# KolinGuo/MPlib

Measured on AMD Instinct MI355X. Metric: configs/sec full collide() Panda-7DoF+10 boxes, higher is better.
Workload: dtype f64; 1 GPU; cfg3 panda_10boxes: 1048576 configs/GPU/step, 129 pairs, full self+world collide() with ACM filter; configs_per_gpu=1048576, pairs=129, mask_words=5, parallelism=dp1 (config shards, no data-path collective)

## Files before the change

### mplib_amd/csrc/mpg_abi_world.h

```cpp
#pragma once

const char* mpg_last_error(void) { return g_last_error.c_str(); }

int mpg_fcl_bvh_build(const double* vertices, int32_t n_vertices, const int32_t* triangles, int32_t n_triangles,
                      double* boxes, int32_t* links, int32_t* leaf_order) {
  if (n_triangles <= 0 || !vertices || !triangles || !boxes || !links || !leaf_order)
    return set_error(MPG_E_INVALID, "mpg_fcl_bvh_build: empty mesh or NULL buffer");
  for (int64_t i = 0; i < 3 * (int64_t)n_triangles; ++i)
    if (triangles[i] < 0 || triangles[i] >= n_vertices) return set_error(MPG_E_INVALID, "triangle vertex out of range");
  FclBvh B;
  B.box.resize(FB_STRIDE);
  B.link.resize(3);
  std::vector<int> prim((size_t)n_triangles);
  for (int t = 0; t < n_triangles; ++t) prim[t] = t;
  fcl_bvh_node(B, vertices, triangles, prim, 0, 0, n_triangles, 0);
  std::copy(B.box.begin(), B.box.end(), boxes);
  std::copy(B.link.begin(), B.link.end(), links);
  std::copy(prim.begin(), prim.end(), leaf_order);
  return (int)(B.link.size() / 3);
}

int mpg_last_error_copy(char* buf, size_t size) {
  const size_t len = g_last_error.size();
  if (buf && size > 0) {
// ... 71 lines not shown

int mpg_synchronize(int device) {
  HIP_TRY(hipSetDevice(device));
  HIP_TRY(hipDeviceSynchronize());
  return MPG_OK;
}

int mpg_world_create(const mpg_world_desc* d_in, int device, mpg_world** out) {
  if (!out) return set_error(MPG_E_INVALID, "out is NULL");
  *out = nullptr;
  int rc = validate(d_in);
  if (rc) return rc;
  mpg_world_desc dd = *d_in;
  std::vector<int32_t> lp_kin(dd.link_parent, dd.link_parent + dd.n_links);
  int n_free = 0;
  for (int32_t& p : lp_kin)
    if (p == MPG_LINK_FREE) {
      p = 0;
      ++n_free;
    }
  if (n_free) dd.link_parent = lp_kin.data();
  const mpg_world_desc* d = &dd;
  std::vector<double> geom_rec((size_t)G_STRIDE * std::max(d->n_geoms, 1), 0.0);
  for (int g = 0; g < d->n_geoms; ++g) geom_record(d, g, geom_rec.data() + (size_t)G_STRIDE * g);
  std::vector<double> obb((size_t)7 * std::max(d->n_geoms, 1), 0.0);
  for (int g = 0; g < d->n_geoms; ++g) {
    const double* r = geom_rec.data() + (size_t)G_STRIDE * g;
    for (int k = 0; k < 3; ++k) obb[7 * g + k] = r[G_OBB_C + k];
    for (int k = 0; k < 3; ++k) obb[7 * g + 3 + k] = r[G_OBB_E + k];
    obb[7 * g + 6] = r[G_RADIUS];
  }
  BpProgram bpp;
  bp_build(d, obb, bpp);
  size_t lds = 0;
  const int W = std::max(1, (d->n_pairs + 31) / 32);
  const int block = choose_block(cull_lds_per_thread(d->n_moving, bpp.n_saves, W), &lds);
  if (block < 0) return set_error(MPG_E_UNSUPPORTED, "world too large for the phase-A LDS budget");
  HIP_TRY(hipSetDevice(device));

  std::vector<double> static_rec((size_t)S_STRIDE * std::max(d->n_static, 1), 0.0);
  for (int s = 0; s < d->n_static; ++s) static_record(d, s, geom_rec.data(), static_rec.data() + (size_t)S_STRIDE * s);
  std::vector<int> gstart(std::max(d->n_geoms, 1), 0), ngroups(std::max(d->n_geoms, 1), 0);
  std::vector<double> hull;
  std::vector<int> cbase(std::max(d->n_geoms, 1), -1), geom_nbr(std::max(d->n_geoms, 1), -1), hull_nbr, wcell_end, wcell_end2, wcell_pre;
  std::vector<double> cell_rec, cell_ovf, wcell_rec, wcell_ovf, wcell_aux, nbr_ent;
  const int walk_subk =
      std::getenv("MPG_WALK_SUBK") ? std::max(1, std::min(8, std::atoi(std::getenv("MPG_WALK_SUBK")))) : kSubK;
  int big_words = 0;
  for (int g = 0; g < d->n_geoms; ++g) {
    if (d->geom_type[g] != MPG_GEOM_CONVEX) continue;
    const double* Vg = d->vertices + 3 * (size_t)d->geom_vertex_start[g];
    const int nvg = d->geom_vertex_count[g];
    std::vector<int> enc;
    const int nf = (int)d->geom_param[4 * g + 1];
    bool walk = nf > 0 && fcl_convex_neighbors(nvg, d->convex_face + (int64_t)d->geom_param[4 * g], nf, enc);
#ifdef MPG_DIAG
    if (std::getenv("MPG_DEBUG_NO_WALK")) walk = false;
#endif
    if (walk) {
      geom_nbr[g] = (int)(hull_nbr.size() / 2);
      if (nvg > kMaxWalkVerts) big_words = std::max(big_words, (nvg + 63) / 64);
      for (int i = 0; i < nvg; ++i) {
        const int st = enc[i], cnt = enc[st];
        hull_nbr.push_back((int)(nbr_ent.size() / 4));
        hull_nbr.push_back(cnt);
        for (int k = 1; k <= cnt; ++k) {
// ... 406 lines not shown
  const size_t o_al = bb.add(allowed.data(), allowed.size());
  const size_t o_cf = bb.add(pair_cf.data(), pair_cf.size());
  const size_t o_sT = bb.add(d->static_transform, 12 * (size_t)d->n_static);
  const size_t o_cs = bb.add(chain_start.data(), chain_start.size());
  const size_t o_cl = bb.add(chain_len.data(), chain_len.size());
  const size_t o_cj = bb.add(chain_joints.data(), chain_joints.size());
  const size_t o_ss = bb.add(sched_start.data(), sched_start.size());
  const size_t o_sp = bb.add(sched_pair.data(), sched_pair.size());
  const size_t o_so = bb.add(sched_other.data(), sched_other.size());
  const size_t o_sts = bb.add(st_start.data(), st_start.size());
  const size_t o_stm = bb.add(st_m.data(), st_m.size());
  const size_t o_str = bb.add(st_r.data(), st_r.size());
  const size_t o_pbd = bb.add(prism_bound.data(), prism_bound.size());
  const size_t o_amk = bb.add(all_mask.data(), all_mask.size());
  const size_t o_bjs = bb.add(bpp.jsrc.data(), bpp.jsrc.size());
  const size_t o_bjv = bb.add(bpp.jsave.data(), bpp.jsave.size());
  const size_t o_bja = bb.add(bpp.jaxis.data(), bpp.jaxis.size());
  const size_t o_bjp = bb.add(bpp.jplace.data(), bpp.jplace.size());
  const size_t o_bls = bb.add(bpp.link_start.data(), bpp.link_start.size());
  const size_t o_blo = bb.add(bpp.link_order.data(), bpp.link_order.size());
  const size_t o_blp = bb.add(bpp.lplace.data(), bpp.lplace.size());
  const size_t o_bos = bb.add(bpp.obj_start.data(), bpp.obj_start.size());
  const size_t o_boo = bb.add(bpp.obj_order.data(), bpp.obj_order.size());
  const size_t o_bmo = bb.add(bpp.moff.data(), bpp.moff.size());
  const size_t o_bmb = bb.add(bpp.mobj.data(), bpp.mobj.size());
  const size_t o_bsb = bb.add(bpp.sobj.data(), bpp.sobj.size());
  if (bpp.jobj_order.empty()) bpp.jobj_order.push_back(0);
  const size_t o_bjk = bb.add(bpp.jkind.data(), bpp.jkind.size());
  const size_t o_bjo = bb.add(bpp.jobj_start.data(), bpp.jobj_start.size());
  const size_t o_bjr = bb.add(bpp.jobj_order.data(), bpp.jobj_order.size());
  const size_t o_bop = bb.add(bpp.oplace.data(), bpp.oplace.size());
  const size_t o_boq = bb.add(bpp.oquat.data(), bpp.oquat.size());
  const size_t o_boc = bb.add(bpp.ocen.data(), bpp.ocen.size());
  const size_t o_olf = bb.add(oct_leaf.data(), oct_leaf.size());
  const size_t o_mtr = bb.add(mesh_tri.data(), mesh_tri.size());
  const size_t o_mnd = bb.add(mesh_node.data(), mesh_node.size());
  const size_t o_mln = bb.add(mesh_link.data(), mesh_link.size());
  const size_t o_mtt = bb.add(mesh_tree.data(), mesh_tree.size());
  const size_t o_lrec = bb.add(lat_rec.data(), lat_rec.size());
  const size_t o_fbb = bb.add(fbvh.box.data(), fbvh.box.size());
  const size_t o_fbl = bb.add(fbvh.link.data(), fbvh.link.size());
  const size_t o_fbr = bb.add(fb_root.data(), fb_root.size());
  const size_t o_tps = bb.add(tri_pos.data(), tri_pos.size());
  const size_t o_sob = bb.add(sobb.data(), sobb.size());
  const size_t o_ogr = bb.add(oct_grid.data(), oct_grid.size());
  const size_t o_oce = bb.add(oct_cells.data(), oct_cells.size());
  const size_t o_oli = bb.add(oct_list.data(), oct_list.size());
  const size_t o_opa = bb.add(oct_path.data(), oct_path.size());
  const size_t o_ode = bb.add(oct_depth.data(), oct_depth.size());
  std::vector<int> free_obj(n_free, 0);
  for (int m = 0; m < d->n_moving; ++m)
    if (d->moving_link[m] >= d->n_links - n_free) free_obj[d->moving_link[m] - (d->n_links - n_free)] = m;
  const size_t o_fob = n_free ? bb.add(free_obj.data(), free_obj.size()) : 0;

  std::unique_ptr<mpg_world> w(new mpg_world());
  w->device = device;
  w->n_geoms = d->n_geoms;
  w->geom_type_h.assign(d->geom_type, d->geom_type + d->n_geoms);
  w->block = block;
  w->lds_bytes = lds;
  w->blob_bytes = bb.bytes.size();
  {
    uint64_t h = 1469598103934665603ull;
    for (const char c : bb.bytes) h = (h ^ (uint8_t)c) * 1099511628211ull;
    w->snapshot_hash = h;
  }
  HIP_TRY(w->blob.reserve(w->blob_bytes));
  HIP_TRY(hipMemcpy(w->blob.get(), bb.bytes.data(), w->blob_bytes, hipMemcpyHostToDevice));
  char* base = w->blob.get();
  DevWorld& dw = w->dw;
  dw.nj = d->n_joints;
  dw.dof = d->dof;
  dw.n_links = d->n_links;
  dw.n_geoms = d->n_geoms;
  dw.n_moving = d->n_moving;
  dw.n_static = d->n_static;
  dw.n_pairs = d->n_pairs;
  dw.W = W;
  dw.mpr_tol = d->gjk_tolerance;
  dw.bp_margin = bp_margin;
  dw.small_margin = small_margin;
  dw.n_prism = n_prism;
  dw.prism_bound = to_cptr<double>(base + o_pbd);
  dw.pose_bound = pose_bound;
  dw.all_mask = to_cptr<int>(base + o_amk);
  dw.n_free = n_free;
  dw.far_r = far_r;
  dw.free_obj = to_cptr<int>(base + o_fob);
  dw.free_cur = nullptr;
  if (n_free) {
    w->free_host.resize((size_t)n_free * 7);
    for (int k = 0; k < n_free; ++k) {
      const double* lp = d->link_placement + 12 * (size_t)(d->n_links - n_free + k);
      double* p7 = w->free_host.data() + 7 * (size_t)k;
      for (int i = 0; i < 3; ++i) p7[i] = lp[9 + i];
      mat_to_quat(lp, &p7[3], &p7[4]);
    }
    HIP_TRY(w->free_dev.reserve(w->free_host.size()));
    HIP_TRY(hipMemcpy(w->free_dev.get(), w->free_host.data(), sizeof(double) * w->free_host.size(),
                      hipMemcpyHostToDevice));
    dw.free_cur = w->free_dev.get();
  }
#ifdef MPG_DIAG
  if (const char* m = std::getenv("MPG_DEBUG_MARGIN")) {
    dw.bp_margin = (float)std::atof(m);
    dw.small_margin = std::atof(m);
  }
#endif
  dw.debug_mode = 0;
#ifdef MPG_DIAG
  if (const char* e = std::getenv("MPG_DEBUG_CULL")) dw.debug_mode = std::atoi(e);
#endif
  dw.big_vis = nullptr;
  dw.big_busy = nullptr;
  dw.big_slots = 0;
  dw.big_words = big_words;
  if (big_words > 0) {
    dw.big_slots = 8192;
    HIP_TRY(w->big_vis.reserve((size_t)dw.big_slots * big_words));
    dw.big_vis = w->big_vis.get();
    HIP_TRY(hipMemset(dw.big_vis, 0, sizeof(unsigned long long) * (size_t)dw.big_slots * big_words));
    HIP_TRY(w->big_busy.reserve((size_t)dw.big_slots));
    dw.big_busy = w->big_busy.get();
    HIP_TRY(hipMemset(dw.big_busy, 0, sizeof(int) * (size_t)dw.big_slots));
  }
  dw.stats = nullptr;
  if (std::getenv("MPG_STATS") && std::atoi(std::getenv("MPG_STATS")) > 0) {
    const size_t n_stats = 64;
    HIP_TRY(w->stats.reserve(n_stats));
    dw.stats = w->stats.get();
    HIP_TRY(hipMemset(dw.stats, 0, n_stats * sizeof(unsigned long long)));
  }
  dw.joint_type = to_cptr<int>(base + o_jt);
  dw.joint_parent = to_cptr<int>(base + o_jp);
  dw.joint_q_source = to_cptr<int>(base + o_jqs);
  dw.joint_q_const = to_cptr<double>(base + o_jqc);
  dw.joint_axis = to_cptr<double>(base + o_ja);
  dw.joint_place = to_cptr<double>(base + o_jpl);
// ... 18 lines not shown
  dw.wcell_end = to_cptr<int>(base + o_wend);
  dw.wcell_end2 = to_cptr<int>(base + o_wend2);
  dw.wcell_pre = to_cptr<int>(base + o_wpre);
  dw.walk_subk = walk_subk;
  dw.moving_link = to_cptr<int>(base + o_ml);
  dw.moving_geom = to_cptr<int>(base + o_mg);
  dw.moving_offset = to_cptr<double>(base + o_mo);
  dw.static_geom = to_cptr<int>(base + o_sg);
  dw.static_rec = to_cptr<double>(base + o_srec);
  dw.pair_a = to_cptr<int>(base + o_pa);
  dw.pair_b = to_cptr<int>(base + o_pb);
  dw.pair_allowed = to_cptr<int>(base + o_al);
  dw.pair_cf = to_cptr<int>(base + o_cf);
  for (int p = 0; p < d->n_pairs; ++p) {
    w->has_closed_form |= pair_cf[p] != CF_NONE && !allowed[p];
    w->has_octree |= pair_cf[p] == CF_OCTREE && !allowed[p];
    w->octree_first |= pair_cf[p] == CF_OCTREE && !allowed[p] && obj_geom_type(d, d->pair_a[p]) == MPG_GEOM_OCTREE;
    w->any_closed_form |= pair_cf[p] != CF_NONE && cf_class(pair_cf[p]) == CLS_CLOSED;
    w->any_octree |= pair_cf[p] == CF_OCTREE;
    w->has_mesh |= pair_cf[p] == CF_MESH && !allowed[p];
    w->any_mesh |= pair_cf[p] == CF_MESH;
    w->any_gjk |= pair_cf[p] == CF_GJK;
    w->has_octree2 |= !allowed[p] && obj_geom_type(d, d->pair_a[p]) == MPG_GEOM_OCTREE &&
                      obj_geom_type(d, d->pair_b[p]) == MPG_GEOM_OCTREE;
  }
  dw.static_T = to_cptr<double>(base + o_sT);
  dw.link_chain_start = to_cptr<int>(base + o_cs);
  dw.link_chain_len = to_cptr<int>(base + o_cl);
  dw.chain_joints = to_cptr<int>(base + o_cj);
  auto I = [&](size_t o) { return to_cptr<int>(base + o); };
  dw.sched_start = I(o_ss);
  dw.sched_pair = I(o_sp);
  dw.sched_other = I(o_so);
  dw.st_start = I(o_sts);
  dw.st_m = I(o_stm);
  dw.st_r = to_cptr<float>(base + o_str);
  auto F = [&](size_t o) { return to_cptr<float>(base + o); };
  BpView& bp = dw.bp;
  bp.nj = d->n_joints;
  bp.n_links = d->n_links;
  bp.n_moving = d->n_moving;
  bp.n_static = d->n_static;
  bp.n_saves = bpp.n_saves;
  bp.joint_type = dw.joint_type;
  bp.joint_q_source = dw.joint_q_source;
  bp.joint_q_const = dw.joint_q_const;
  bp.jsrc = I(o_bjs);
  bp.jsave = I(o_bjv);
  bp.jaxis = F(o_bja);
  bp.jplace = F(o_bjp);
  bp.link_start = I(o_bls);
  bp.link_order = I(o_blo);
  bp.lplace = F(o_blp);
  bp.obj_start = I(o_bos);
  bp.obj_order = I(o_boo);
  bp.moving_link = dw.moving_link;
  bp.moff = F(o_bmo);
  bp.mobj = F(o_bmb);
  bp.sobj = F(o_bsb);
  bp.jkind = I(o_bjk);
  bp.jobj_start = I(o_bjo);
  bp.jobj_order = I(o_bjr);
  bp.oplace = F(o_bop);
  bp.oquat = F(o_boq);
  bp.ocen = F(o_boc);
  dw.oct_leaf = to_cptr<double>(base + o_olf);
  dw.oct_path = to_cptr<uint64_t>(base + o_opa);
  dw.oct_depth = to_cptr<int>(base + o_ode);
  dw.mesh_tri = to_cptr<double>(base + o_mtr);
  dw.mesh_node = to_cptr<double>(base + o_mnd);
  dw.mesh_link = to_cptr<int>(base + o_mln);
  dw.mesh_tree = to_cptr<int>(base + o_mtt);
  dw.fb_box = to_cptr<double>(base + o_fbb);
  dw.fb_link = to_cptr<int>(base + o_fbl);
  dw.fb_root = to_cptr<int>(base + o_fbr);
  dw.tri_pos = to_cptr<int>(base + o_tps);
  dw.sobb = to_cptr<double>(base + o_sob);
  dw.lat_rec = to_cptr<double>(base + o_lrec);
  dw.lat_rec_ok = lat_rec_ok ? 1 : 0;
  dw.oct_grid = to_cptr<double>(base + o_ogr);
  dw.oct_cells = I(o_oce);
  dw.oct_list = I(o_oli);
  int cus = 256;
  if (hipDeviceGetAttribute(&cus, hipDeviceAttributeMultiprocessorCount, device) != hipSuccess || cus <= 0) cus = 256;
  int per_cu = 0;
  if (hipOccupancyMaxActiveBlocksPerMultiprocessor(&per_cu, narrow_kernel<false>, 256, 0) != hipSuccess || per_cu <= 0)
    per_cu = 2;
  w->narrow_blocks = cus * per_cu;
  {
    auto& K = w->ik;
    K.cus = cus;
    K.chain_start = chain_start;
    K.chain_len = chain_len;
    K.chain_joints = chain_joints;
    K.joint_q_source.assign(d->joint_q_source, d->joint_q_source + d->n_joints);
    const size_t nd = (size_t)std::max(d->dof, 0);
    K.lo.assign(nd, -INFINITY);
    K.hi.assign(nd, INFINITY);
// ... 118 lines not shown
```

### mplib_amd/csrc/mpg_broadphase.h

```cpp
#pragma once
#include <cmath>
#include <vector>

#include "mpg_math.h"
#include "../../include/mpgpu.h"

namespace mpg {

constexpr float kBpMargin = 1e-4f;
constexpr double kFp32CullRel = 4e-6;
constexpr float kFarPark = 1e15f;
constexpr double kFreeQuatTol = 1e-6;
constexpr double kDefaultTravel = 10.0;

#ifdef __clang__
#define MPG_FP32_CONTRACT _Pragma("clang fp contract(fast)")
#else
#define MPG_FP32_CONTRACT
#endif

enum { BM_C = 0, BM_E = 3, BM_R = 6, BM_STRIDE = 8 };
enum { BS_C = 0, BS_R = 3, BS_E = 12, BS_STRIDE = 16 };

struct BpView {
  int nj, n_links, n_moving, n_static, n_saves;
  cptr<int> joint_type;
  cptr<int> joint_q_source;
  cptr<double> joint_q_const;
  cptr<int> jsrc;
  cptr<int> jsave;
  cptr<float> jaxis;
  cptr<float> jplace;
  cptr<int> link_start;
  cptr<int> link_order;
  cptr<float> lplace;
  cptr<int> obj_start;
  cptr<int> obj_order;
  cptr<int> moving_link;
  cptr<float> moff;
  cptr<float> mobj;
  cptr<float> sobj;
  cptr<int> jkind;
  cptr<int> jobj_start;
  cptr<int> jobj_order;
  cptr<float> oplace;
  cptr<float> oquat;
  cptr<float> ocen;
};

enum BpKind { BK_FIXED = 0, BK_REV_X = 1, BK_REV_AXIS = 4, BK_PRI_X = 5, BK_PRI_AXIS = 8, BK_SKIP = 9 };

struct F34 {
  float R[9];
  float p[3];
};

template <class P>
MPG_INLINE F34 f34_load(P a) {
  F34 T;
#pragma unroll
  for (int i = 0; i < 9; ++i) T.R[i] = a[i];
  T.p[0] = a[9];
  T.p[1] = a[10];
  T.p[2] = a[11];
  return T;
}

MPG_INLINE F34 f34_mul(const F34& A, const F34& B) {
  MPG_FP32_CONTRACT
  F34 C;
#pragma unroll
  for (int i = 0; i < 3; ++i) {
#pragma unroll
    for (int j = 0; j < 3; ++j)
      C.R[3 * i + j] = A.R[3 * i] * B.R[j] + A.R[3 * i + 1] * B.R[3 + j] + A.R[3 * i + 2] * B.R[6 + j];
    C.p[i] = A.R[3 * i] * B.p[0] + A.R[3 * i + 1] * B.p[1] + A.R[3 * i + 2] * B.p[2] + A.p[i];
  }
  return C;
}

// ... 245 lines not shown
}

#ifdef __clang__
typedef float mpg_f2 __attribute__((ext_vector_type(2)));
template <class P>
MPG_INLINE uint32_t fsphere_obb_keep2(const float* c, float r, P rec, float margin) {
  MPG_FP32_CONTRACT
  auto ld = [&](int k) { return mpg_f2{rec[2 * k], rec[2 * k + 1]}; };
  const mpg_f2 d0 = c[0] - ld(BS_C), d1 = c[1] - ld(BS_C + 1), d2 = c[2] - ld(BS_C + 2);
  mpg_f2 acc = {0.f, 0.f};
#pragma unroll
  for (int j = 0; j < 3; ++j) {
    const mpg_f2 t = d0 * ld(BS_R + j) + d1 * ld(BS_R + 3 + j) + d2 * ld(BS_R + 6 + j);
    const mpg_f2 a = mpg_f2{fabsf(t.x), fabsf(t.y)} - ld(BS_E + j);
    const mpg_f2 ex = mpg_f2{fmaxf(a.x, 0.f), fmaxf(a.y, 0.f)};
    acc += ex * ex;
  }
  const float rr = r + margin;
  const float r2 = rr * rr;
  return (uint32_t)!(acc.x > r2) | ((uint32_t)!(acc.y > r2) << 1);
}
#else
template <class P>
inline uint32_t fsphere_obb_keep2(const float* c, float r, P rec, float margin) {
  float a[BS_STRIDE], b[BS_STRIDE];
  for (int k = 0; k < BS_STRIDE; ++k) {
    a[k] = rec[2 * k];
    b[k] = rec[2 * k + 1];
  }
  return (uint32_t)!fsphere_obb_separated(c, r, a, margin) | ((uint32_t)!fsphere_obb_separated(c, r, b, margin) << 1);
}
#endif

struct BpProgram {
  int n_saves = 0;
  std::vector<int> jsrc, jsave, link_start, link_order, obj_start, obj_order, jkind, jobj_start, jobj_order;
  std::vector<float> jaxis, jplace, lplace, moff, mobj, sobj, oplace, oquat, ocen;
};

inline void se3d_mul(const double* A, const double* B, double* C) {
  double T[12];
  for (int i = 0; i < 3; ++i) {
    for (int j = 0; j < 3; ++j) T[3 * i + j] = A[3 * i] * B[j] + A[3 * i + 1] * B[3 + j] + A[3 * i + 2] * B[6 + j];
    T[9 + i] = A[3 * i] * B[9] + A[3 * i + 1] * B[10] + A[3 * i + 2] * B[11] + A[9 + i];
  }
  for (int k = 0; k < 12; ++k) C[k] = T[k];
}

inline void mat_to_quat_d(const double* m, double* q) {
  const double d[4] = {1.0 + m[0] + m[4] + m[8], 1.0 + m[0] - m[4] - m[8], 1.0 - m[0] + m[4] - m[8],
                       1.0 - m[0] - m[4] + m[8]};
  int k = 0;
  for (int i = 1; i < 4; ++i)
    if (d[i] > d[k]) k = i;
  const double h = 0.5 * std::sqrt(d[k]), s = 0.25 / h;
  if (k == 0) {
    q[3] = h; q[0] = (m[7] - m[5]) * s; q[1] = (m[2] - m[6]) * s; q[2] = (m[3] - m[1]) * s;
  } else if (k == 1) {
    q[0] = h; q[3] = (m[7] - m[5]) * s; q[1] = (m[1] + m[3]) * s; q[2] = (m[2] + m[6]) * s;
  } else if (k == 2) {
    q[1] = h; q[3] = (m[2] - m[6]) * s; q[0] = (m[1] + m[3]) * s; q[2] = (m[5] + m[7]) * s;
  } else {
    q[2] = h; q[3] = (m[3] - m[1]) * s; q[0] = (m[2] + m[6]) * s; q[1] = (m[5] + m[7]) * s;
  }
}

inline void joint_motion_d(int type, const double* axis, double v, double* M) {
  for (int k = 0; k < 12; ++k) M[k] = (k == 0 || k == 4 || k == 8) ? 1.0 : 0.0;
  if (type <= MPG_JOINT_REVOLUTE_UNALIGNED || type >= MPG_JOINT_RUBX) {
    const double s = std::sin(v), c = std::cos(v);
// ... 96 lines not shown
      if (ojoint[m] == j) P.jobj_order.push_back(m);
  }
  P.jobj_start[nj + 1] = (int)P.jobj_order.size();
  P.oquat.assign((size_t)4 * std::max(nm, 1), 0.f);
  P.ocen.assign((size_t)3 * std::max(nm, 1), 0.f);
  for (int m = 0; m < nm; ++m) {
    const double* O = ofold.data() + 12 * m;
    for (int k = 0; k < 12; ++k) P.oplace[12 * m + k] = (float)O[k];
    double q[4];
    mat_to_quat_d(O, q);
    for (int k = 0; k < 4; ++k) P.oquat[4 * m + k] = (float)q[k];
    const double* g = obb.data() + 7 * d->moving_geom[m];
    for (int i = 0; i < 3; ++i)
      P.ocen[3 * m + i] = (float)(O[3 * i] * g[0] + O[3 * i + 1] * g[1] + O[3 * i + 2] * g[2] + O[9 + i]);
  }
  P.mobj.assign((size_t)BM_STRIDE * std::max(nm, 1), 0.f);
  for (int m = 0; m < nm; ++m) {
    const double* g = obb.data() + 7 * d->moving_geom[m];
    float* r = P.mobj.data() + BM_STRIDE * m;
    for (int k = 0; k < 3; ++k) r[BM_C + k] = (float)g[k];
    for (int k = 0; k < 3; ++k) r[BM_E + k] = widen(g[3 + k]);
    r[BM_R] = widen(g[6]);
  }
  P.sobj.assign((size_t)BS_STRIDE * std::max(ns, 1), 0.f);
  for (int s = 0; s < ns; ++s) {
    const double* T = d->static_transform + 12 * s;
    const double* g = obb.data() + 7 * d->static_geom[s];
    float* r = P.sobj.data() + BS_STRIDE * s;
    for (int i = 0; i < 3; ++i)
      r[BS_C + i] = (float)(T[3 * i] * g[0] + T[3 * i + 1] * g[1] + T[3 * i + 2] * g[2] + T[9 + i]);
    for (int k = 0; k < 9; ++k) r[BS_R + k] = (float)T[k];
    for (int k = 0; k < 3; ++k) r[BS_E + k] = widen(g[3 + k]);
  }
}

inline BpView bp_view(const mpg_world_desc* d, const BpProgram& P) {
  BpView b{};
  b.nj = d->n_joints;
  b.n_links = d->n_links;
  b.n_moving = d->n_moving;
  b.n_static = d->n_static;
  b.n_saves = P.n_saves;
  b.joint_type = to_cptr<int>(d->joint_type);
  b.joint_q_source = to_cptr<int>(d->joint_q_source);
  b.joint_q_const = to_cptr<double>(d->joint_q_const);
  b.jsrc = to_cptr<int>(P.jsrc.data());
  b.jsave = to_cptr<int>(P.jsave.data());
  b.jaxis = to_cptr<float>(P.jaxis.data());
  b.jplace = to_cptr<float>(P.jplace.data());
  b.link_start = to_cptr<int>(P.link_start.data());
  b.link_order = to_cptr<int>(P.link_order.data());
  b.lplace = to_cptr<float>(P.lplace.data());
  b.obj_start = to_cptr<int>(P.obj_start.data());
  b.obj_order = to_cptr<int>(P.obj_order.data());
  b.moving_link = to_cptr<int>(d->moving_link);
  b.moff = to_cptr<float>(P.moff.data());
  b.mobj = to_cptr<float>(P.mobj.data());
  b.sobj = to_cptr<float>(P.sobj.data());
  b.jkind = to_cptr<int>(P.jkind.data());
  b.jobj_start = to_cptr<int>(P.jobj_start.data());
  b.jobj_order = to_cptr<int>(P.jobj_order.data());
  b.oplace = to_cptr<float>(P.oplace.data());
  b.oquat = to_cptr<float>(P.oquat.data());
  b.ocen = to_cptr<float>(P.ocen.data());
  return b;
}

}
```

### mplib_amd/csrc/mpg_fk.h

```cpp
#pragma once
#include "mpg_math.h"
#include "mpg_broadphase.h"
#include "mpg_hullcells.h"
#include "../../include/mpgpu.h"

namespace mpg {

constexpr int kMaxJoints = 32;

enum { G_PARAM = 0, G_INTERIOR = 4, G_OBB_C = 7, G_OBB_E = 10, G_RADIUS = 13, G_VMAX = 14, G_AABB_E = 15, G_STRIDE = 18 };
enum { S_ROT = 0, S_ROTINV = 4, S_POS = 8, S_OBBC = 11, S_R = 14, S_STRIDE = 23 };

struct DevWorld {
  int nj, dof, n_links, n_geoms, n_moving, n_static, n_pairs, W;
  double mpr_tol;
  float bp_margin;
  double small_margin;
  int debug_mode;
  unsigned long long* stats;
  MPG_INLINE bool dbg(int k) const {
#ifdef MPG_DIAG
    return debug_mode == k;
#else
    (void)k;
    return false;
#endif
  }
  cptr<int> joint_type;
  cptr<int> joint_parent;
  cptr<int> joint_q_source;
  cptr<double> joint_q_const;
  cptr<double> joint_axis;
  cptr<double> joint_place;
  cptr<int> link_parent;
  cptr<double> link_place;
  cptr<int> geom_type;
  cptr<int> geom_gstart;
  cptr<int> geom_ng;
  cptr<int> geom_nvert;
  cptr<double> geom_rec;
  cptr<double> hull;
  int hull_doubles;
  cptr<int> geom_cbase;
  cptr<double> cell_rec;
  cptr<double> cell_ovf;
  cptr<int> geom_nbr;
  cptr<int> hull_nbr;
  cptr<double> nbr_ent;
  cptr<double> wcell_rec;
  cptr<double> wcell_ovf;
  cptr<double> wcell_aux;
  cptr<int> wcell_end;
  cptr<int> wcell_end2;
  cptr<int> wcell_pre;
  int walk_subk;
  cptr<int> moving_link;
  cptr<int> moving_geom;
  cptr<double> moving_offset;
  cptr<int> static_geom;
  cptr<double> static_rec;
  cptr<int> pair_a;
  cptr<int> pair_b;
  cptr<int> pair_allowed;
  cptr<int> pair_cf;
  cptr<double> static_T;
  cptr<int> link_chain_start;
  cptr<int> link_chain_len;
  cptr<int> chain_joints;
  BpView bp;
  cptr<int> sched_start;
  cptr<int> sched_pair;
  cptr<int> sched_other;
  cptr<int> st_start;
  cptr<int> st_m;
  cptr<float> st_r;
  int n_prism;
  cptr<double> prism_bound;
  double pose_bound;
  cptr<int> all_mask;
  unsigned long long* big_vis;
  int* big_busy;
  int big_slots, big_words;
  cptr<double> oct_leaf;
  cptr<double> oct_grid;
  cptr<int> oct_cells;
  cptr<int> oct_list;
  cptr<uint64_t> oct_path;
  cptr<int> oct_depth;
  cptr<double> mesh_tri;
  cptr<double> mesh_node;
  cptr<int> mesh_link;
  cptr<int> mesh_tree;
  cptr<double> fb_box;
  cptr<int> fb_link;
  cptr<int> fb_root;
  cptr<int> tri_pos;
  cptr<double> sobb;
  cptr<double> lat_rec;
  int lat_rec_ok;
  int n_free;
  cptr<int> free_obj;
  const double* free_cur;
  double far_r;
};
constexpr int kLatChain = 12;
// ... 113 lines not shown
```

### mplib_amd/csrc/mpg_kernels.hip

```cpp

#include <hip/hip_runtime.h>

#include <algorithm>
#include <atomic>
#include <chrono>
#include <cfloat>
#include <cstdio>
#include <cstdlib>
#include <cstring>
#include <limits>
#include <map>
#include <memory>
#include <mutex>
#include <string>
#include <thread>
#include <vector>

#include "../../include/mpgpu.h"
#include "mpg_math.h"
#include "mpg_fk.h"
#include "mpg_ik.h"
#include "mpg_screw.h"
#include "mpg_bucket.h"
#include "mpg_hostpipe.h"
// ... 846 lines not shown
    if (lane >= (uint32_t)off) v += u;
  }
  return v;
}

template <int BLOCK>
__device__ __forceinline__ FObb bp_obb(const DevWorld& w, const float* __restrict__ cen, const float* __restrict__ rq,
                                       long long cap, int id, int t, long long cfg) {
  FObb o;
  if (id < w.n_moving) {
    const float* q = rq + (size_t)id * 4 * cap + cfg;
    f_quat_to_mat(q[3 * cap], q[0], q[cap], q[2 * cap], o.R);
    const float* c = cen + (size_t)id * 3 * BLOCK + t;
    o.c[0] = c[0];
    o.c[1] = c[BLOCK];
    o.c[2] = c[2 * BLOCK];
    const cptr<float> g = w.bp.mobj + BM_STRIDE * id;
    o.e[0] = g[BM_E];
    o.e[1] = g[BM_E + 1];
    o.e[2] = g[BM_E + 2];
  } else {
    const cptr<float> g = w.bp.sobj + BS_STRIDE * (id - w.n_moving);
#pragma unroll
    for (int k = 0; k < 3; ++k) o.c[k] = g[BS_C + k];
#pragma unroll
    for (int k = 0; k < 9; ++k) o.R[k] = g[BS_R + k];
#pragma unroll
    for (int k = 0; k < 3; ++k) o.e[k] = g[BS_E + k];
  }
  return o;
}

template <int BLOCK>
__device__ __forceinline__ void sat_drain(const DevWorld& w, const float* __restrict__ cen, const float* __restrict__ rq,
                                          long long cap, long long cfg0, uint32_t* survw, const uint32_t* queue,
                                          uint32_t head, uint32_t cnt, int wbase, uint32_t lane) {
  __builtin_amdgcn_wave_barrier();
  if (lane < cnt) {
    const uint32_t e = queue[(head + lane) & (kQueue - 1)];
    const int p = w.sched_pair[(int)(e >> 6)], t = wbase + (int)(e & 63u);
    const FObb A = bp_obb<BLOCK>(w, cen, rq, cap, w.pair_a[p], t, cfg0 + t);
    const FObb B = bp_obb<BLOCK>(w, cen, rq, cap, w.pair_b[p], t, cfg0 + t);
    if (!fobb_separated(A, B, w.bp_margin)) atomicOr(&survw[(p >> 5) * BLOCK + t], 1u << (p & 31));
  }
  __builtin_amdgcn_wave_barrier();
}

template <int BLOCK, bool FROM_POSES>
__global__ __launch_bounds__(BLOCK) void cull_kernel(DevWorld w, const double* __restrict__ in, long long n,
                                                    uint8_t* __restrict__ flags, uint32_t* __restrict__ masks,
                                                    uint32_t* __restrict__ surv, float* __restrict__ rq,
                                                    double* __restrict__ sc, long long cap,
                                                    uint32_t* __restrict__ cnt, int n_tiles) {
  extern __shared__ __attribute__((aligned(16))) float lds_f[];
  float* cen = lds_f;
  float* save = cen + (size_t)w.n_moving * 3 * BLOCK;
  uint32_t* survw = reinterpret_cast<uint32_t*>(save + (size_t)max(w.bp.n_saves - kRegSaves, 0) * 12 * BLOCK);
  const int tid = threadIdx.x;
  uint32_t* queue = survw + (size_t)w.W * BLOCK + (tid >> 6) * kQueue;
  const uint32_t lane = lane_id();
  const int wbase = tid & ~63;
  const long long cfg0 = (long long)blockIdx.x * BLOCK;
  const long long cfg = cfg0 + tid;
  const bool live = cfg < n;
  const long long c = live ? cfg : n - 1;
  if (live) {
    flags[cfg] = 0;
    if (masks)
      for (int k = 0; k < w.W; ++k) masks[cfg * w.W + k] = 0u;
  }
  for (int k = 0; k < w.W; ++k) survw[k * BLOCK + tid] = 0u;
  if (w.dbg(14)) return;

  auto store_obj = [&](int m, const float* q, const float* c) {
    if (live && !w.dbg(13)) {
      float* r = rq + (size_t)m * 4 * cap + cfg;
#pragma unroll
      for (int k = 0; k < 4; ++k) r[k * cap] = q[k];
    }
    float* r = cen + (size_t)m * 3 * BLOCK + tid;
#pragma unroll
    for (int i = 0; i < 3; ++i) r[i * BLOCK] = c[i];
// ... 26 lines not shown
      forced |= !(std::fabs(pl[0]) <= w.pose_bound && std::fabs(pl[1]) <= w.pose_bound && std::fabs(pl[2]) <= w.pose_bound);
    }
    for (int k = 0; k < w.n_free; ++k) {
      const double* pl = in + (c * w.n_links + nk + k) * 7;
      const int m = w.free_obj[k];
      const cptr<double> gr = w.geom_rec + G_STRIDE * w.moving_geom[m];
      double R[9];
      quat_to_mat(pl[3], pl[4], pl[5], pl[6], R);
      double d2 = 0.0;
#pragma unroll
      for (int i = 0; i < 3; ++i) {
        const double ci = R[3 * i] * gr[G_OBB_C] + R[3 * i + 1] * gr[G_OBB_C + 1] + R[3 * i + 2] * gr[G_OBB_C + 2] + pl[i];
        d2 += ci * ci;
      }
      if (std::sqrt(d2) - gr[G_RADIUS] > w.far_r) {
        float* r = cen + (size_t)m * 3 * BLOCK + tid;
        r[0] = kFarPark;
        r[BLOCK] = 0.f;
        r[2 * BLOCK] = 0.f;
      }
    }
  } else {
    bp_fk(w.bp, in + c * w.dof, save + tid, BLOCK, put_j);
    if (w.n_prism)
      for (int j = 0; j < w.nj; ++j)
        if (w.prism_bound[j] >= 0.0) forced |= !(std::fabs(in[c * w.dof + w.joint_q_source[j]]) <= w.prism_bound[j]);
  }
  if (w.dbg(1) || w.dbg(13)) {
    if (live && cen[tid] == 12345.f) flags[cfg] = 2;
    return;
  }

  uint32_t head = 0, tail = 0;
  uint32_t dbg_keep = 0u;
  auto push = [&](int eb, uint32_t kb) {
    if (!live) kb = 0u;
    if (w.dbg(11)) {
      dbg_keep += kb;
      return;
    }
    if (w.dbg(2)) {
      for (int i = 0; i < 32; ++i) {
        if (!((kb >> i) & 1u)) continue;
        const int p = w.sched_pair[eb + i];
        survw[(p >> 5) * BLOCK + tid] |= 1u << (p & 31);
      }
      return;
    }
    {
    const uint32_t c = (uint32_t)__popc(kb);
    uint32_t ex = 0u, total = 0u;
#pragma unroll
    for (int bit = 0; bit < 6; ++bit) {
      const unsigned long long m = __ballot((c >> bit) & 1u);
      ex += __builtin_amdgcn_mbcnt_hi((uint32_t)(m >> 32), __builtin_amdgcn_mbcnt_lo((uint32_t)m, 0u)) << bit;
      total += (uint32_t)__popcll(m) << bit;
    }
    const uint32_t incl = ex + c;
    if (total == 0u) return;
    if (tail - head + total <= (uint32_t)kQueue) {
      uint32_t pos = tail + incl - c;
      while (kb) {
        const int i = __builtin_ctz(kb);
        kb &= kb - 1u;
        queue[pos++ & (kQueue - 1)] = ((uint32_t)(eb + i) << 6) | lane;
      }
      tail += total;
      while (tail - head >= 64) {
        sat_drain<BLOCK>(w, cen, rq, cap, cfg0, survw, queue, head, 64, wbase, lane);
        head += 64;
      }
      return;
    }
    }
    uint32_t any_kb = kb;
#pragma unroll
    for (int sh = 1; sh < 64; sh <<= 1) any_kb |= (uint32_t)__shfl_xor((int)any_kb, sh);
    any_kb = __builtin_amdgcn_readfirstlane(any_kb);
    while (any_kb) {
      const int i = __builtin_ctz(any_kb);
      any_kb &= any_kb - 1u;
      const bool keep = (kb >> i) & 1u;
      const unsigned long long bal = __ballot(keep);
      if (keep) {
        const uint32_t rank =
            __builtin_amdgcn_mbcnt_hi((uint32_t)(bal >> 32), __builtin_amdgcn_mbcnt_lo((uint32_t)bal, 0u));
        queue[(tail + rank) & (kQueue - 1)] = ((uint32_t)(eb + i) << 6) | lane;
      }
      tail += (uint32_t)__popcll(bal);
      if (tail - head >= 64) {
        sat_drain<BLOCK>(w, cen, rq, cap, cfg0, survw, queue, head, 64, wbase, lane);
        head += 64;
      }
    }
  };
  const int ns = w.n_static;
  for (int g = 0; g < (FROM_POSES ? 2 : 1) && !w.dbg(12); ++g) {
    const int E0 = w.st_start[g * (ns + 1)], E1 = w.st_start[g * (ns + 1) + ns];
    if (E0 == E1) continue;
    int eb = E0;
    uint32_t kb = 0u;
    for (int sid = 0; sid < ns; ++sid) {
      const int e0 = w.st_start[g * (ns + 1) + sid], e1 = w.st_start[g * (ns + 1) + sid + 1];
      if (e0 == e1) continue;
      const cptr<float> rec = w.bp.sobj + BS_STRIDE * sid;
      float sr[BS_STRIDE];
#pragma unroll
      for (int k = 0; k < BS_STRIDE; ++k) sr[k] = rec[k];
#pragma unroll 2
      for (int e = e0; e < e1; ++e) {
        if (e - eb == 32) {
          push(eb, kb);
          eb = e;
          kb = 0u;
        }
        const float* rm = cen + (size_t)w.st_m[e] * 3 * BLOCK + tid;
        const float cm[3] = {rm[0], rm[BLOCK], rm[2 * BLOCK]};
        kb |= (uint32_t)!fsphere_obb_separated(cm, w.st_r[e], sr, w.bp_margin) << (e - eb);
      }
    }
    push(eb, kb);
  }
  for (int m = 0; m < w.n_moving; ++m) {
    const int e0 = w.sched_start[m], e1 = w.sched_start[m + 1];
    if (e0 == e1) continue;
    const float* rm = cen + (size_t)m * 3 * BLOCK + tid;
    const float cm[3] = {rm[0], rm[BLOCK], rm[2 * BLOCK]};
    const float r_m = w.bp.mobj[BM_STRIDE * m + BM_R];
    for (int eb = e0; eb < e1; eb += 32) {
      const int ee = min(e1, eb + 32);
      uint32_t kb = 0u;
#pragma unroll 4
      for (int e = eb; e < ee; ++e) {
        const int o = w.sched_other[e];
        const float* ro = cen + (size_t)o * 3 * BLOCK + tid;
        const float dx = ro[0] - cm[0], dy = ro[BLOCK] - cm[1], dz = ro[2 * BLOCK] - cm[2];
        const float rr = r_m + w.bp.mobj[BM_STRIDE * o + BM_R] + w.bp_margin;
        kb |= (uint32_t)(dx * dx + dy * dy + dz * dz <= rr * rr) << (e - eb);
      }
      push(eb, kb);
    }
  }
  if (tail != head) sat_drain<BLOCK>(w, cen, rq, cap, cfg0, survw, queue, head, tail - head, wbase, lane);
  if (forced)
    for (int k = 0; k < w.W; ++k) survw[k * BLOCK + tid] = (uint32_t)w.all_mask[k];
  if (w.dbg(8) || w.dbg(11)) {
    if (live && (survw[tid] == 12345u || dbg_keep == 12345u)) flags[cfg] = 2;
    return;
  }
  bool any = false;
  const long long tile = bk_wave_tile(blockIdx.x, BLOCK, tid);
  const bool has_row = bk_tile_has_row(tile, n_tiles);
  if (w.W * 8 <= kQueue) {
    uint32_t* hist = queue;
    for (int i = (int)lane; i < w.W * 8; i += 64) hist[i] = 0u;
    wave_lds_sync();
    for (int k = 0; k < w.W; ++k) {
      uint32_t x = live ? survw[k * BLOCK + tid] : 0u;
      if (live) surv[(long long)k * cap + cfg] = x;
      any |= x != 0u;
      while (x) {
        const int p = k * 32 + __builtin_ctz(x);
        x &= x - 1u;
        atomicAdd(&hist[p >> 2], 1u << (8 * (p & 3)));
      }
    }
    wave_lds_sync();
    if (has_row) {
      uint32_t* row = cnt + tile * bk_row_words(w.W);
      for (int i = (int)lane; i < bk_row_words(w.W); i += 64) row[i] = hist[i];
    }
  } else {
    for (int k = 0; k < w.W; ++k) {
      uint32_t x = live ? survw[k * BLOCK + tid] : 0u;
      if (live) surv[(long long)k * cap + cfg] = x;
      any |= x != 0u;
// ... 5107 lines not shown
```

Measured before the change: 1.597 billion configs/s.

## Add support-height table cull stage after OBB SAT in broadphase

Adds a second broadphase filter: for convex geoms the host precomputes a cube-map table of support heights, and pairs that survive the OBB SAT test are compacted across the wave and checked with tighter support-function separating axes before being marked as survivors. The aim is to cut the number of pairs passed to the expensive narrowphase. Pair metadata is packed into a single sched_rec record, and the cull kernel gets a waves_per_eu(4,4) occupancy hint. The cost is extra per-pair work and register pressure in the cull kernel, and the fp32 interpolation margin has to stay conservative.

```diff
diff --git a/mplib_amd/csrc/mpg_abi_world.h b/mplib_amd/csrc/mpg_abi_world.h
--- a/mplib_amd/csrc/mpg_abi_world.h
+++ b/mplib_amd/csrc/mpg_abi_world.h
@@ -127,6 +127,7 @@
   }
   BpProgram bpp;
   bp_build(d, obb, bpp);
+  bp_build_support(d, obb, bpp);
   size_t lds = 0;
   const int W = std::max(1, (d->n_pairs + 31) / 32);
   const int block = choose_block(cull_lds_per_thread(d->n_moving, bpp.n_saves, W), &lds);
@@ -599,6 +600,17 @@
   const size_t o_bop = bb.add(bpp.oplace.data(), bpp.oplace.size());
   const size_t o_boq = bb.add(bpp.oquat.data(), bpp.oquat.size());
   const size_t o_boc = bb.add(bpp.ocen.data(), bpp.ocen.size());
+  const size_t o_bsh = bb.add(bpp.shtab.data(), bpp.shtab.size());
+  std::vector<int> sched_rec(SR_STRIDE * sched_pair.size(), 0);
+  for (size_t e = 0; e < sched_pair.size() && d->n_pairs > 0; ++e) {
+    const int p = sched_pair[e];
+    int* r = sched_rec.data() + SR_STRIDE * e;
+    r[SR_P] = p;
+    r[SR_A] = d->pair_a[p];
+    r[SR_B] = d->pair_b[p];
+    r[SR_SH] = (bpp.pair_sh[2 * p] + 2) | ((bpp.pair_sh[2 * p + 1] + 2) << 16);
+  }
+  const size_t o_srr = bb.add(sched_rec.data(), sched_rec.size());
   const size_t o_olf = bb.add(oct_leaf.data(), oct_leaf.size());
   const size_t o_mtr = bb.add(mesh_tri.data(), mesh_tri.size());
   const size_t o_mnd = bb.add(mesh_node.data(), mesh_node.size());
@@ -646,6 +658,7 @@
   dw.W = W;
   dw.mpr_tol = d->gjk_tolerance;
   dw.bp_margin = bp_margin;
+  dw.sh_margin = bp_margin + (float)(kFp32CullRel * X);
   dw.small_margin = small_margin;
   dw.n_prism = n_prism;
   dw.prism_bound = to_cptr<double>(base + o_pbd);
@@ -671,6 +684,7 @@
 #ifdef MPG_DIAG
   if (const char* m = std::getenv("MPG_DEBUG_MARGIN")) {
     dw.bp_margin = (float)std::atof(m);
+    dw.sh_margin = dw.bp_margin + (float)(kFp32CullRel * X);
     dw.small_margin = std::atof(m);
   }
 #endif
@@ -755,6 +769,7 @@
   dw.sched_start = I(o_ss);
   dw.sched_pair = I(o_sp);
   dw.sched_other = I(o_so);
+  dw.sched_rec = I(o_srr);
   dw.st_start = I(o_sts);
   dw.st_m = I(o_stm);
   dw.st_r = to_cptr<float>(base + o_str);
@@ -787,6 +802,7 @@
   bp.oplace = F(o_bop);
   bp.oquat = F(o_boq);
   bp.ocen = F(o_boc);
+  bp.shtab = F(o_bsh);
   dw.oct_leaf = to_cptr<double>(base + o_olf);
   dw.oct_path = to_cptr<uint64_t>(base + o_opa);
   dw.oct_depth = to_cptr<int>(base + o_ode);
diff --git a/mplib_amd/csrc/mpg_broadphase.h b/mplib_amd/csrc/mpg_broadphase.h
--- a/mplib_amd/csrc/mpg_broadphase.h
+++ b/mplib_amd/csrc/mpg_broadphase.h
@@ -46,6 +46,7 @@
   cptr<float> oplace;
   cptr<float> oquat;
   cptr<float> ocen;
+  cptr<float> shtab;
 };
 
 enum BpKind { BK_FIXED = 0, BK_REV_X = 1, BK_REV_AXIS = 4, BK_PRI_X = 5, BK_PRI_AXIS = 8, BK_SKIP = 9 };
@@ -357,10 +358,97 @@
 }
 #endif
 
+#if defined(__HIP_DEVICE_COMPILE__)
+#define MPG_SCHED_FENCE __builtin_amdgcn_sched_barrier(0)
+#else
+#define MPG_SCHED_FENCE (void)0
+#endif
+constexpr int kShK = 8;
+constexpr int kShN = kShK + 1;
+constexpr int kShFloats = 6 * kShN * kShN;
+enum { SH_NONE = -1, SH_SKIP = -2 };
+enum { SR_P = 0, SR_A = 1, SR_B = 2, SR_SH = 3, SR_STRIDE = 4 };
+
+template <class P>
+MPG_INLINE float bp_support_height(P tab, float x, float y, float z) {
+  MPG_FP32_CONTRACT
+  const float ax = fabsf(x), ay = fabsf(y), az = fabsf(z);
+  int f;
+  float m, u, v;
+  if (ax >= ay && ax >= az) {
+    f = 0; m = x; u = y; v = z;
+  } else if (ay >= az) {
+    f = 1; m = y; u = z; v = x;
+  } else {
+    f = 2; m = z; u = x; v = y;
+  }
+  const float am = fabsf(m);
+#if defined(__HIP_DEVICE_COMPILE__)
+  const float inv = __builtin_amdgcn_rcpf(am);
+#else
+  const float inv = 1.0f / am;
+#endif
+  const float hk = 0.5f * kShK;
+  const float fu = fminf(fmaxf((u * inv + 1.0f) * hk, 0.f), (float)kShK);
+  const float fv = fminf(fmaxf((v * inv + 1.0f) * hk, 0.f), (float)kShK);
+  int iu = (int)fu, iv = (int)fv;
+  iu = iu > kShK - 1 ? kShK - 1 : iu;
+  iv = iv > kShK - 1 ? kShK - 1 : iv;
+  const float tu = fu - (float)iu, tv = fv - (float)iv;
+  const P c = tab + ((2 * f + (m < 0.f ? 1 : 0)) * kShN + iu) * kShN + iv;
+  const float h00 = c[0], h01 = c[1], h10 = c[kShN], h11 = c[kShN + 1];
+  const float a = h00 + tv * (h01 - h00), b = h10 + tv * (h11 - h10);
+  return (a + tu * (b - a)) * am;
+}
+
+template <class P>
+MPG_INLINE bool bp_support_separated(const FObb& A, const FObb& B, int ta, int tb, P tab, float margin) {
+  MPG_FP32_CONTRACT
+  const float d[3] = {B.c[0] - A.c[0], B.c[1] - A.c[1], B.c[2] - A.c[2]};
+  float Rm[3][3], t[3], s[3];
+#pragma unroll
+  for (int i = 0; i < 3; ++i) {
+#pragma unroll
+    for (int j = 0; j < 3; ++j) Rm[i][j] = A.R[i] * B.R[j] + A.R[3 + i] * B.R[3 + j] + A.R[6 + i] * B.R[6 + j];
+    t[i] = d[0] * A.R[i] + d[1] * A.R[3 + i] + d[2] * A.R[6 + i];
+    s[i] = d[0] * B.R[i] + d[1] * B.R[3 + i] + d[2] * B.R[6 + i];
+  }
+  const float dd = d[0] * d[0] + d[1] * d[1] + d[2] * d[2];
+  float ha = A.e[0] * fabsf(t[0]) + A.e[1] * fabsf(t[1]) + A.e[2] * fabsf(t[2]);
+  float hb = B.e[0] * fabsf(s[0]) + B.e[1] * fabsf(s[1]) + B.e[2] * fabsf(s[2]);
+  bool sep = false;
+  if (ta >= 0) {
+    const P tA = tab + (size_t)ta * kShFloats;
+    ha = bp_support_height(tA, t[0], t[1], t[2]);
+#pragma unroll
+    for (int j = 0; j < 3; ++j) {
+      if (j == 1) MPG_SCHED_FENCE;
+      const float sg = s[j] < 0.f ? -1.f : 1.f;
+      const float h = bp_support_height(tA, sg * Rm[0][j], sg * Rm[1][j], sg * Rm[2][j]);
+      sep |= fabsf(s[j]) - h - B.e[j] > margin;
+    }
+  }
+  if (tb >= 0) {
+    const P tB = tab + (size_t)tb * kShFloats;
+    hb = bp_support_height(tB, -s[0], -s[1], -s[2]);
+#pragma unroll
+    for (int i = 0; i < 3; ++i) {
+      if (i == 1) MPG_SCHED_FENCE;
+      const float sg = t[i] < 0.f ? 1.f : -1.f;
+      const float h = bp_support_height(tB, sg * Rm[i][0], sg * Rm[i][1], sg * Rm[i][2]);
+      sep |= fabsf(t[i]) - A.e[i] - h > margin;
+    }
+  }
+  sep |= dd - ha - hb > margin * sqrtf(dd);
+  return sep;
+}
+
 struct BpProgram {
   int n_saves = 0;
   std::vector<int> jsrc, jsave, link_start, link_order, obj_start, obj_order, jkind, jobj_start, jobj_order;
   std::vector<float> jaxis, jplace, lplace, moff, mobj, sobj, oplace, oquat, ocen;
+  std::vector<float> shtab;
+  std::vector<int> pair_sh;
 };
 
 inline void se3d_mul(const double* A, const double* B, double* C) {
@@ -523,6 +611,48 @@
     for (int k = 0; k < 9; ++k) r[BS_R + k] = (float)T[k];
     for (int k = 0; k < 3; ++k) r[BS_E + k] = widen(g[3 + k]);
   }
+}
+
+inline void bp_support_table(const double* V, int nv, const double* c, float* tab) {
+  for (int f = 0; f < 3; ++f)
+    for (int sgn = 0; sgn < 2; ++sgn)
+      for (int i = 0; i < kShN; ++i)
+        for (int j = 0; j < kShN; ++j) {
+          double dir[3];
+          dir[f] = sgn ? -1.0 : 1.0;
+          dir[(f + 1) % 3] = -1.0 + 2.0 * i / kShK;
+          dir[(f + 2) % 3] = -1.0 + 2.0 * j / kShK;
+          double h = -INFINITY;
+          for (int k = 0; k < nv; ++k)
+            h = std::max(h, (V[3 * k] - c[0]) * dir[0] + (V[3 * k + 1] - c[1]) * dir[1] + (V[3 * k + 2] - c[2]) * dir[2]);
+          tab[((2 * f + sgn) * kShN + i) * kShN + j] = widen(h);
+        }
+}
+
+inline void bp_build_support(const mpg_world_desc* d, const std::vector<double>& obb, BpProgram& P) {
+  std::vector<int> gtab(std::max(d->n_geoms, 1), SH_NONE);
+  auto table_of = [&](int g) {
+    const int t = d->geom_type[g];
+    if (t == MPG_GEOM_MESH || t == MPG_GEOM_OCTREE) return (int)SH_SKIP;
+    if (t != MPG_GEOM_CONVEX || d->geom_vertex_count[g] <= 0) return (int)SH_NONE;
+    if (gtab[g] < 0) {
+      gtab[g] = (int)(P.shtab.size() / kShFloats);
+      P.shtab.resize(P.shtab.size() + kShFloats);
+      bp_support_table(d->vertices + 3 * (size_t)d->geom_vertex_start[g], d->geom_vertex_count[g], obb.data() + 7 * g,
+                       P.shtab.data() + (size_t)gtab[g] * kShFloats);
+    }
+    return gtab[g];
+  };
+  auto geom_of = [&](int id) { return id < d->n_moving ? d->moving_geom[id] : d->static_geom[id - d->n_moving]; };
+  P.pair_sh.assign(2 * (size_t)std::max(d->n_pairs, 1), SH_SKIP);
+  for (int p = 0; p < d->n_pairs; ++p) {
+    if (d->pair_allowed && d->pair_allowed[p]) continue;
+    const int ta = table_of(geom_of(d->pair_a[p])), tb = table_of(geom_of(d->pair_b[p]));
+    if (ta == SH_SKIP || tb == SH_SKIP || (ta < 0 && tb < 0)) continue;
+    P.pair_sh[2 * p] = ta;
+    P.pair_sh[2 * p + 1] = tb;
+  }
+  if (P.shtab.empty()) P.shtab.assign(kShFloats, 0.f);
 }
 
 inline BpView bp_view(const mpg_world_desc* d, const BpProgram& P) {
@@ -554,6 +684,7 @@
   b.oplace = to_cptr<float>(P.oplace.data());
   b.oquat = to_cptr<float>(P.oquat.data());
   b.ocen = to_cptr<float>(P.ocen.data());
+  b.shtab = to_cptr<float>(P.shtab.data());
   return b;
 }
 
diff --git a/mplib_amd/csrc/mpg_fk.h b/mplib_amd/csrc/mpg_fk.h
--- a/mplib_amd/csrc/mpg_fk.h
+++ b/mplib_amd/csrc/mpg_fk.h
@@ -15,6 +15,7 @@
   int nj, dof, n_links, n_geoms, n_moving, n_static, n_pairs, W;
   double mpr_tol;
   float bp_margin;
+  float sh_margin;
   double small_margin;
   int debug_mode;
   unsigned long long* stats;
@@ -71,6 +72,7 @@
   cptr<int> sched_start;
   cptr<int> sched_pair;
   cptr<int> sched_other;
+  cptr<int> sched_rec;
   cptr<int> st_start;
   cptr<int> st_m;
   cptr<float> st_r;
diff --git a/mplib_amd/csrc/mpg_kernels.hip b/mplib_amd/csrc/mpg_kernels.hip
--- a/mplib_amd/csrc/mpg_kernels.hip
+++ b/mplib_amd/csrc/mpg_kernels.hip
@@ -902,22 +902,58 @@
 }
 
 template <int BLOCK>
+__device__ __forceinline__ void support_drain(const DevWorld& w, const float* __restrict__ cen, const float* __restrict__ rq,
+                                           long long cap, long long cfg0, uint32_t* survw, uint32_t e, uint32_t cnt,
+                                           int wbase, uint32_t lane) {
+  if (lane < cnt) {
+    const cptr<int> r = w.sched_rec + SR_STRIDE * (int)(e >> 6);
+    const int p = r[SR_P], sh = r[SR_SH], t = wbase + (int)(e & 63u);
+    const FObb A = bp_obb<BLOCK>(w, cen, rq, cap, r[SR_A], t, cfg0 + t);
+    const FObb B = bp_obb<BLOCK>(w, cen, rq, cap, r[SR_B], t, cfg0 + t);
+    if (!bp_support_separated(A, B, (sh & 0xffff) - 2, (sh >> 16) - 2, w.bp.shtab, w.sh_margin))
+      atomicOr(&survw[(p >> 5) * BLOCK + t], 1u << (p & 31));
+  }
+}
+
+template <int BLOCK>
 __device__ __forceinline__ void sat_drain(const DevWorld& w, const float* __restrict__ cen, const float* __restrict__ rq,
                                           long long cap, long long cfg0, uint32_t* survw, const uint32_t* queue,
-                                          uint32_t head, uint32_t cnt, int wbase, uint32_t lane) {
+                                          uint32_t head, uint32_t cnt, int wbase, uint32_t lane, uint32_t& pend,
+                                          uint32_t& npend) {
   __builtin_amdgcn_wave_barrier();
+  uint32_t e = 0u;
+  bool keep = false;
   if (lane < cnt) {
-    const uint32_t e = queue[(head + lane) & (kQueue - 1)];
-    const int p = w.sched_pair[(int)(e >> 6)], t = wbase + (int)(e & 63u);
-    const FObb A = bp_obb<BLOCK>(w, cen, rq, cap, w.pair_a[p], t, cfg0 + t);
-    const FObb B = bp_obb<BLOCK>(w, cen, rq, cap, w.pair_b[p], t, cfg0 + t);
-    if (!fobb_separated(A, B, w.bp_margin)) atomicOr(&survw[(p >> 5) * BLOCK + t], 1u << (p & 31));
+    e = queue[(head + lane) & (kQueue - 1)];
+    const cptr<int> r = w.sched_rec + SR_STRIDE * (int)(e >> 6);
+    const int p = r[SR_P], sh = r[SR_SH], t = wbase + (int)(e & 63u);
+    const FObb A = bp_obb<BLOCK>(w, cen, rq, cap, r[SR_A], t, cfg0 + t);
+    const FObb B = bp_obb<BLOCK>(w, cen, rq, cap, r[SR_B], t, cfg0 + t);
+    if (!fobb_separated(A, B, w.bp_margin)) {
+      if ((sh & 0xffff) == SH_SKIP + 2) atomicOr(&survw[(p >> 5) * BLOCK + t], 1u << (p & 31));
+      else keep = true;
+    }
+  }
+  const unsigned long long bal = __ballot(keep);
+  const uint32_t ns = (uint32_t)__popcll(bal);
+  if (ns) {
+    const uint32_t rank = __builtin_amdgcn_mbcnt_hi((uint32_t)(bal >> 32), __builtin_amdgcn_mbcnt_lo((uint32_t)bal, 0u));
+    const uint32_t dst = keep ? npend + rank : npend + ns + (lane - rank);
+    const uint32_t recv = (uint32_t)__builtin_amdgcn_ds_permute((int)((dst & 63u) << 2), (int)e);
+    if (npend + ns >= 64u) {
+      support_drain<BLOCK>(w, cen, rq, cap, cfg0, survw, lane >= npend ? recv : pend, 64, wbase, lane);
+      pend = recv;
+      npend = npend + ns - 64u;
+    } else {
+      if (lane >= npend && lane < npend + ns) pend = recv;
+      npend += ns;
+    }
   }
   __builtin_amdgcn_wave_barrier();
 }
 
 template <int BLOCK, bool FROM_POSES>
-__global__ __launch_bounds__(BLOCK) void cull_kernel(DevWorld w, const double* __restrict__ in, long long n,
+__global__ __launch_bounds__(BLOCK) __attribute__((amdgpu_waves_per_eu(4, 4))) void cull_kernel(DevWorld w, const double* __restrict__ in, long long n,
                                                     uint8_t* __restrict__ flags, uint32_t* __restrict__ masks,
                                                     uint32_t* __restrict__ surv, float* __restrict__ rq,
                                                     double* __restrict__ sc, long long cap,
@@ -1010,6 +1046,7 @@
   }
 
   uint32_t head = 0, tail = 0;
+  uint32_t pend = 0u, npend = 0u;
   uint32_t dbg_keep = 0u;
   auto push = [&](int eb, uint32_t kb) {
     if (!live) kb = 0u;
@@ -1045,7 +1082,7 @@
       }
       tail += total;
       while (tail - head >= 64) {
-        sat_drain<BLOCK>(w, cen, rq, cap, cfg0, survw, queue, head, 64, wbase, lane);
+        sat_drain<BLOCK>(w, cen, rq, cap, cfg0, survw, queue, head, 64, wbase, lane, pend, npend);
         head += 64;
       }
       return;
@@ -1067,7 +1104,7 @@
       }
       tail += (uint32_t)__popcll(bal);
       if (tail - head >= 64) {
-        sat_drain<BLOCK>(w, cen, rq, cap, cfg0, survw, queue, head, 64, wbase, lane);
+        sat_drain<BLOCK>(w, cen, rq, cap, cfg0, survw, queue, head, 64, wbase, lane, pend, npend);
         head += 64;
       }
     }
@@ -1119,7 +1156,9 @@
       push(eb, kb);
     }
   }
-  if (tail != head) sat_drain<BLOCK>(w, cen, rq, cap, cfg0, survw, queue, head, tail - head, wbase, lane);
+  if (tail != head) sat_drain<BLOCK>(w, cen, rq, cap, cfg0, survw, queue, head, tail - head, wbase, lane, pend, npend);
+  if (npend) support_drain<BLOCK>(w, cen, rq, cap, cfg0, survw, pend, npend, wbase, lane);
+  __builtin_amdgcn_wave_barrier();
   if (forced)
     for (int k = 0; k < w.W; ++k) survw[k * BLOCK + tid] = (uint32_t)w.all_mask[k];
   if (w.dbg(8) || w.dbg(11)) {
```

New measurement: 1.655 billion configs/s (median of 6 runs). 1.04x the previous value.
